# IBM/VillanDiffusion

Measured on AMD Instinct MI355X. Metric: train imgs/sec + 1000-step DDPM sample imgs/sec, CIFAR10 bs128, higher is better.
Workload: dtype bf16x3/f32

## Files before the change

### villandiffusion_amd/csrc/vd_gemm.hip

```cpp
#include "vd_common.h"
#include <string.h>
#include <stdlib.h>

bool vd_conv3_k32p_eligible(const vd_gemm_desc& d);
int vd_launch_conv3_k32p(const vd_gemm_desc& d, int mode, hipStream_t st);
int vd_launch_wgrad_ps_group(const void* jobs, int n, int W, int up, int blocks, hipStream_t st, bool one);
bool vd_conv3_sm_eligible(const vd_gemm_desc& d);
int vd_launch_conv3_sm(const vd_gemm_desc& d, hipStream_t st);
bool vd_gemm1x1_k32p_pick(const vd_gemm_desc& d);
int vd_launch_gemm1x1_k32p(const vd_gemm_desc& d, hipStream_t st);

namespace {

constexpr int NT = 256;
constexpr int BK = 32;
constexpr int KG = BK / 4;

struct Pix {
    int b, oy, ox, p;
    bool valid;
};

__device__ __forceinline__ void kdecomp9(int k, int& c, int& r, int& s) {
    c = k / 9;
// ... 881 lines not shown
                    float v = acc[m][j];
#pragma unroll
                    for (int k = 0; k < NW - 1; ++k) v += red[k][m][j][lane];
                    v *= d.alpha;
                    if (d.bias) v += d.bias[m];
                    o[j] = v;
                }
                *reinterpret_cast<f32x4*>(d.D + (int64_t)b * d.d_bstride + (int64_t)m * d.ldd + y * W + 4 * x4) = o;
            }
        }
    }
}

static bool fewout_eligible(const vd_gemm_desc& d) {
    return d.W % 4 == 0 && d.C >= 16 && (d.b_bstride & 3) == 0 && (d.d_bstride & 3) == 0 && (d.ldd & 3) == 0 &&
           ((((uintptr_t)d.B) | ((uintptr_t)d.D)) & 15) == 0 && (int64_t)d.H * d.W == d.NP;
}

static bool smallm_eligible(const vd_gemm_desc& d) {
    if (d.b_mode == VD_B_CONV3_T) {
        if (d.a_mode != VD_A_ROW || d.M > 4 || d.tile != 0 || d.debug != 0 || d.act || d.bias || d.pool2 || d.b_presplit) return false;
        if (d.rowadd || d.residual || d.d_trans || d.accumulate || d.bias_on_n || d.nb2 > 1 || d.a_bstride != 0 || d.gn_ss) return false;
        return d.OH == d.H && d.OW == d.W && d.lda == d.K && d.K == d.C * 9 && fewout_eligible(d);
    }
    if (d.b_mode != VD_B_CONV3 || d.a_mode != VD_A_ROW || d.M > 4 || d.tile != 0 || d.debug != 0 || d.act) return false;
    if (d.rowadd || d.residual || d.d_trans || d.accumulate || d.bias_on_n || d.nb2 > 1 || d.a_bstride != 0 || d.gn_ss) return false;
    if (d.OH != d.H || d.OW != d.W) return false;
    if (d.W % 32 == 0) return d.H % 8 == 0;
    return d.W == 16 && d.H % 16 == 0;
}

static int launch_smallm(const vd_gemm_desc& d, hipStream_t st) {
    const int nb = d.N / d.NP;
    if (d.b_mode == VD_B_CONV3_T) {
        const int64_t quads = (int64_t)nb * d.H * (d.W / 4);
        hipLaunchKernelGGL((conv3_fewout_kernel<4, 8, true>), dim3((unsigned)((quads + 63) / 64)), dim3(512), 0, st, d, quads);
        return 0;
    }
    if (fewout_eligible(d)) {
        const int64_t quads = (int64_t)nb * d.H * (d.W / 4);
        hipLaunchKernelGGL((conv3_fewout_kernel<4, 8>), dim3((unsigned)((quads + 63) / 64)), dim3(512), 0, st, d, quads);
        return 0;
    }
    if (d.W % 32 == 0) {
        dim3 grid((unsigned)(nb * (d.H / 8) * (d.W / 32)));
        hipLaunchKernelGGL((conv3_smallm_kernel<32, 4>), grid, dim3(256), 0, st, d);
    } else {
        dim3 grid((unsigned)(nb * (d.H / 16)));
        hipLaunchKernelGGL((conv3_smallm_kernel<16, 4>), grid, dim3(256), 0, st, d);
    }
    return 0;
}

template <int AMODE>
__global__ __launch_bounds__(NT, 3) void gemm_plain_kernel(const vd_gemm_desc d) {
    constexpr int WM = 2, WN = 2, BM = 128, BN = 128;
    constexpr int LD_ = 128 + 4;
    constexpr int LDA_ = (AMODE == VD_A_ROW) ? 129 : 132;
    constexpr int F4 = BM * BK / 4 / NT;
    __shared__ __attribute__((aligned(16))) float As[BK * LDA_];
    __shared__ __attribute__((aligned(16))) float Bs[BK * LD_];

    const int tid = threadIdx.x, lane = tid & 63, wave = tid >> 6, h = lane >> 5;
    const int tiles_m = (d.M + BM - 1) / BM;
    int bid = blockIdx.x;
    {
        const int nwg = gridDim.x;
        if ((nwg & 7) == 0) bid = (bid & 7) * (nwg >> 3) + (bid >> 3);
    }
    const int tm = bid % tiles_m, tn = bid / tiles_m;
    const int m0 = tm * BM, n0 = tn * BN;
    const int b = n0 / d.NP, p0 = n0 - b * d.NP;
    const float* __restrict__ Ap = d.A + batch_off(d, b, d.a_bstride, d.a_b2stride);
    const float* __restrict__ Bp = d.B + batch_off(d, b, d.b_bstride, d.b_b2stride) + p0;

    f32x4 ra[F4], rb[F4];
    auto load_stage = [&](int k0) {
#pragma unroll
        for (int i = 0; i < F4; ++i) {
            const int idx = tid + i * NT;
            if (AMODE == VD_A_ROW) {
                const int m = idx >> 3, q = idx & 7;
                ra[i] = *reinterpret_cast<const f32x4*>(Ap + (int64_t)min(m0 + m, d.M - 1) * d.lda + k0 + 4 * q);
            } else {
                const int k = idx >> 5, q = idx & 31;
                ra[i] = *reinterpret_cast<const f32x4*>(Ap + (int64_t)(k0 + k) * d.lda + min(m0 + 4 * q, d.M - 4));
            }
            const int k = idx >> 5, q = idx & 31;
            rb[i] = *reinterpret_cast<const f32x4*>(Bp + (int64_t)(k0 + k) * d.ldb + 4 * q);
        }
    };
    auto store_stage = [&]() {
#pragma unroll
        for (int i = 0; i < F4; ++i) {
            const int idx = tid + i * NT;
            if (AMODE == VD_A_ROW) {
                const int m = idx >> 3, q = idx & 7;
                const bool ok = m0 + m < d.M;
#pragma unroll
                for (int j = 0; j < 4; ++j) As[(4 * q + j) * LDA_ + m] = ok ? ra[i][j] : 0.f;
            } else {
                const int k = idx >> 5, q = idx & 31;
                const bool ok = m0 + 4 * q < d.M;
                *reinterpret_cast<f32x4*>(&As[k * LDA_ + 4 * q]) = ok ? ra[i] : f32x4{0.f, 0.f, 0.f, 0.f};
            }
            const int k = idx >> 5, q = idx & 31;
// ... 768 lines not shown
    if (row >= B * M) return;
    const int b = row / M, m = row - b * M;
    const float* __restrict__ x = X + (int64_t)b * x_bs + (int64_t)m * P;
    const int lane = threadIdx.x & 63;
    float s = 0.f;
    if ((P & 3) == 0 && ((((uintptr_t)x) & 15) == 0)) {
        const f32x4* x4 = reinterpret_cast<const f32x4*>(x);
        const int Q = P >> 2;
        int i = lane;
        for (; i + 192 < Q; i += 256) {
            const f32x4 v0 = x4[i], v1 = x4[i + 64], v2 = x4[i + 128], v3 = x4[i + 192];
            s += (v0[0] + v0[1]) + (v0[2] + v0[3]);
            s += (v1[0] + v1[1]) + (v1[2] + v1[3]);
            s += (v2[0] + v2[1]) + (v2[2] + v2[3]);
            s += (v3[0] + v3[1]) + (v3[2] + v3[3]);
        }
        for (; i < Q; i += 64) {
            f32x4 v = x4[i];
            s += (v[0] + v[1]) + (v[2] + v[3]);
        }
    } else {
        for (int i = lane; i < P; i += 64) s += x[i];
    }
    s = wave_sum(s);
    if (lane == 0) ws[(int64_t)b * ws_ld + m] = s;
}

__global__ __launch_bounds__(256) void colsum_kernel(const float* __restrict__ ws, float* __restrict__ out, int B, int C,
                                                     int64_t ld, int accumulate) {
    __shared__ float part[4][64];
    const int lane = threadIdx.x & 63, w = threadIdx.x >> 6;
    const int c = blockIdx.x * 64 + lane;
    float s = 0.f;
    if (c < C) {
        int b = w;
        for (; b + 28 < B; b += 32) {
            float t[8];
#pragma unroll
            for (int u = 0; u < 8; ++u) t[u] = ws[(int64_t)(b + 4 * u) * ld + c];
#pragma unroll
            for (int u = 0; u < 8; ++u) s += t[u];
        }
        for (; b < B; b += 4) s += ws[(int64_t)b * ld + c];
    }
    part[w][lane] = s;
    __syncthreads();
    if (w == 0 && c < C) {
        const float t = (part[0][lane] + part[1][lane]) + (part[2][lane] + part[3][lane]);
        out[c] = accumulate ? (out[c] + t) : t;
    }
}

template <bool BIG_IS_X>
__global__ __launch_bounds__(256) void wgrad_small_kernel(const vd_wgrad_desc d) {
    constexpr int MAXS = 4, PWM = 34;
    __shared__ float S[MAXS * PWM * PWM];
    const int CB = BIG_IS_X ? d.C : d.M, CS = BIG_IS_X ? d.M : d.C;
    const int H = d.OH, W = d.OW, HW = H * W;
    constexpr int PW = PWM, PHW = PWM * PWM;
    const int cb_blocks = (CB + 31) / 32, tiles_x = (W + 31) / 32, tiles = tiles_x * ((H + 31) / 32);
    int rest = blockIdx.x;
    const int cb0 = (rest % cb_blocks) * 32;
    rest /= cb_blocks;
    const int tile = rest % tiles, b = rest / tiles;
    const int y0 = (tile / tiles_x) * 32, x0 = (tile - (tile / tiles_x) * tiles_x) * 32;
    const int TH = min(32, H - y0), TW = min(32, W - x0);
    const float* __restrict__ big = (BIG_IS_X ? d.X + (int64_t)b * d.x_bstride : d.dY + (int64_t)b * d.dy_bstride);
    const float* __restrict__ sml = (BIG_IS_X ? d.dY + (int64_t)b * d.dy_bstride : d.X + (int64_t)b * d.x_bstride);
    for (int i = threadIdx.x; i < CS * PHW; i += 256) {
        const int cs = i / PHW, rem = i - cs * PHW;
        const int yy = y0 + rem / PW - 1, xx = x0 + rem - (rem / PW) * PW - 1;
        const bool ok = (unsigned)yy < (unsigned)H && (unsigned)xx < (unsigned)W;
        S[i] = ok ? sml[(int64_t)cs * HW + yy * W + xx] : 0.f;
    }
    __syncthreads();
    const int x = threadIdx.x & 31, slot = threadIdx.x >> 5;
    const int Ncols = d.C * 9;
    float* __restrict__ part = d.ws + ((int64_t)b * tiles + tile) * d.M * Ncols;
    float acc[4][MAXS][9];
#pragma unroll
    for (int k = 0; k < 4; ++k)
#pragma unroll
        for (int cs = 0; cs < MAXS; ++cs)
#pragma unroll
            for (int t = 0; t < 9; ++t) acc[k][cs][t] = 0.f;
    if (x < TW) {
        const float* __restrict__ src[4];
        bool live[4];
#pragma unroll
        for (int k = 0; k < 4; ++k) {
            const int cb = cb0 + slot + 8 * k;
            live[k] = cb < CB;
            src[k] = big + (int64_t)(live[k] ? cb : 0) * HW + (int64_t)y0 * W + x0 + x;
        }
        for (int y = 0; y < TH; ++y) {
            float v[4];
#pragma unroll
            for (int k = 0; k < 4; ++k) v[k] = src[k][y * W];
#pragma unroll
            for (int k = 0; k < 4; ++k) v[k] = live[k] ? v[k] : 0.f;
#pragma unroll
            for (int cs = 0; cs < MAXS; ++cs) {
                if (cs < CS) {
                    const float* __restrict__ sp = S + cs * PHW + (y + 1) * PW + (x + 1);
#pragma unroll
                    for (int t = 0; t < 9; ++t) {
                        const int r = t / 3, sx = t - 3 * r;
                        const int dy = BIG_IS_X ? 1 - r : r - 1, dx = BIG_IS_X ? 1 - sx : sx - 1;
                        const float sv = sp[dy * PW + dx];
#pragma unroll
                        for (int k = 0; k < 4; ++k) acc[k][cs][t] = fmaf(v[k], sv, acc[k][cs][t]);
                    }
                }
            }
        }
    }
#pragma unroll
    for (int k = 0; k < 4; ++k) {
        const int cb = cb0 + slot + 8 * k;
        if (cb >= CB) continue;
#pragma unroll
        for (int cs = 0; cs < MAXS; ++cs) {
            if (cs < CS) {
#pragma unroll
                for (int t = 0; t < 9; ++t) {
                    float v = acc[k][cs][t];
#pragma unroll
                    for (int off = 16; off > 0; off >>= 1) v += __shfl_xor(v, off, 32);
                    if (x == 0) {
                        const int m = BIG_IS_X ? cs : cb, c = BIG_IS_X ? cb : cs;
                        part[(int64_t)m * Ncols + c * 9 + t] = v;
                    }
                }
            }
        }
    }
}

static bool wgrad_small_eligible(const vd_wgrad_desc& d) {
    if (d.T != 9 || d.mode != VD_B_CONV3 || d.tile != 0 || d.math != 0) return false;
    if (d.H != d.OH || d.W != d.OW || d.OH * d.OW != d.NP) return false;
    const bool small_m = d.M <= 4 && d.C >= 32, small_c = d.C <= 4 && d.M >= 32;
    return (small_m || small_c) && d.nb >= 1;
}
static int wgrad_small_parts(const vd_wgrad_desc& d) { return d.nb * vd_cdiv(d.OW, 32) * vd_cdiv(d.OH, 32); }

__global__ __launch_bounds__(256) void colsum_seg_kernel(const int64_t* __restrict__ table, int B) {
    __shared__ float part[4][64];
    const int64_t* __restrict__ t = table + 4 * (int64_t)blockIdx.x;
    const float* __restrict__ ws = reinterpret_cast<const float*>(t[0]);
    float* __restrict__ out = reinterpret_cast<float*>(t[1]);
    const int C = (int)t[2];
    const int64_t ld = t[3];
    const int lane = threadIdx.x & 63, w = threadIdx.x >> 6;
    const int c = lane;
    float s = 0.f;
    if (c < C) {
        int b = w;
        for (; b + 28 < B; b += 32) {
            float v[8];
#pragma unroll
            for (int u = 0; u < 8; ++u) v[u] = ws[(int64_t)(b + 4 * u) * ld + c];
#pragma unroll
            for (int u = 0; u < 8; ++u) s += v[u];
        }
        for (; b < B; b += 4) s += ws[(int64_t)b * ld + c];
    }
    part[w][lane] = s;
    __syncthreads();
    if (w == 0 && c < C) out[c] += (part[0][lane] + part[1][lane]) + (part[2][lane] + part[3][lane]);
}

template <int WM, int WN>
int launch_gemm_t(const vd_gemm_desc& d, hipStream_t st) {
    constexpr int BM = 64 * WM, BN = 64 * WN;
    const int grid = vd_cdiv(d.M, BM) * vd_cdiv(d.N, BN);
#define VD_GEMM_CASE(AM, BMD)                                                                   \
    if (d.a_mode == AM && d.b_mode == BMD) {                                                    \
        hipLaunchKernelGGL((gemm_kernel<WM, WN, AM, BMD>), dim3(grid), dim3(NT), 0, st, d);     \
        return 0;                                                                               \
    }
    VD_GEMM_CASE(VD_A_ROW, VD_B_PLAIN)
    VD_GEMM_CASE(VD_A_ROW, VD_B_KCONTIG)
    VD_GEMM_CASE(VD_A_ROW, VD_B_CONV3)
    VD_GEMM_CASE(VD_A_ROW, VD_B_CONV3_T)
    VD_GEMM_CASE(VD_A_ROW, VD_B_CONV3_S2)
    VD_GEMM_CASE(VD_A_ROW, VD_B_CONV3_UP)
    VD_GEMM_CASE(VD_A_ROW, VD_B_CONV3_DIL)
    VD_GEMM_CASE(VD_A_ROW, VD_B_CONVG)
    VD_GEMM_CASE(VD_A_COL, VD_B_PLAIN)
    VD_GEMM_CASE(VD_A_COL, VD_B_KCONTIG)
// ... 35 lines not shown
    unsigned long long* p = (unsigned long long*)buf;
    return (int)hipMemcpyToSymbol(HIP_SYMBOL(g_wg_stamps), &p, sizeof(p));
}
#endif

extern "C" int64_t vd_gemm_ws_floats(const vd_gemm_desc* desc) {
    if (desc && desc->a_packed) {
        const int tile = vd_gemm_tile(desc);
        int splits = 1, per;
        if (tile == 9) gemm_bx3_plan(*desc, splits, per);
        else if (tile == 8 || tile == 16) bx3_plan(*desc, splits, per);
        return splits > 1 ? (int64_t)splits * desc->M * desc->N : 0;
    }
    if (!desc || !patch_eligible(*desc)) return 0;
    int splits, ks_per;
    patch_plan(*desc, splits, ks_per);
    return splits > 1 ? (int64_t)splits * desc->M * desc->N : 0;
}

extern "C" int vd_gemm_tile(const vd_gemm_desc* desc) {
    if (!desc) return 0;
    const vd_gemm_desc& d = *desc;
    if (d.a_packed && d.math == 2) {
        if (bx3_eligible(d) && !bx3_big_split(d) && k32p_pick(d)) return 18;
        if (gemm_bx3_eligible(d) && vd_gemm1x1_k32p_pick(d)) return 19;
        return -1;
    }
    if (d.a_packed && d.math == 3) {
        if (bx3_eligible(d)) {
            if (vd_conv3_sm_eligible(d)) return 20;
            if (!bx3_big_split(d) && k32p_pick(d)) return 18;
            return -1;
        }
        if (gemm_bx3_eligible(d) && vd_gemm1x1_k32p_pick(d)) return 19;
        return -1;
    }
    if (d.a_packed) {
        if (bx3_eligible(d)) {
            if (vd_conv3_sm_eligible(d)) return 20;
            if (bx3_big_split(d)) return 16;
            if (k32p_pick(d)) return 18;
            int splits, c_per;
            bx3_plan(d, splits, c_per);
            const int big = d.b_mode == VD_B_CONV3_S2 ? 0 : bx3_big_tile(d, splits);
            return big == 2 ? 15 : (big == 1 ? 12 : 8);
        }
        if (!gemm_bx3_eligible(d)) return -1;
        if (vd_gemm1x1_k32p_pick(d)) return 19;
        if (gemm_bx3_big_tile(d)) return 13;
        return vd_cdiv(d.M, 128) * (d.N / 128) >= 1024 ? 11 : 9;
    }
    if (d.math == 1) return gemm_bx3_act_eligible(d) ? 10 : -1;
    if (smallm_eligible(d)) return 7;
    if (patch_eligible(d)) {
        int splits, ks_per;
        patch_plan(d, splits, ks_per);
        return (splits == 1 && patch_wide(d)) ? 6 : 4;
    }
    if (plain_eligible(d)) return 5;
    int max_bn = 128;
    if (d.a_bstride != 0 && d.NP % 128 != 0) max_bn = 64;
    int tile = d.tile ? d.tile : pick_tile(d.M, d.N, max_bn);
    if (max_bn < 128 && tile != 3) tile = 3;
    return tile;
}

extern "C" int vd_gemm(const vd_gemm_desc* desc, void* stream) {
    VD_REQUIRE(desc != nullptr, "vd_gemm: null desc");
    vd_gemm_desc d = *desc;
    VD_REQUIRE(d.A && d.B && d.D, "vd_gemm: null operand");
    VD_REQUIRE(d.math != 3 || d.a_packed, "vd_gemm: math = 3 (one bf16 product per term) reads the hi plane of a_packed; a_packed is NULL");
#ifndef VD_ABLATION
    VD_REQUIRE(d.debug == 0, "vd_gemm: desc.debug = %d -- timing-only ablation bits exist in `make ABLATION=1` builds only", d.debug);
#endif
    VD_REQUIRE(d.M > 0 && d.N > 0 && d.K > 0 && d.NP > 0 && d.N % d.NP == 0, "vd_gemm: bad dims M=%d N=%d K=%d NP=%d", d.M,
               d.N, d.K, d.NP);
    if (d.b_mode >= VD_B_CONV3) {
        VD_REQUIRE(d.C > 0 && d.H > 0 && d.W > 0 && d.OH * d.OW == d.NP, "vd_gemm: bad conv dims");
        if (d.b_mode == VD_B_CONVG)
            VD_REQUIRE(d.kh > 0 && d.kw > 0 && d.K == d.C * d.kh * d.kw && d.conv_stride >= 1 && d.conv_stride <= 4 && d.pad_h >= 0 && d.pad_w >= 0 &&
                           d.OH == (d.H + 2 * d.pad_h - d.kh) / d.conv_stride + 1 && d.OW == (d.W + 2 * d.pad_w - d.kw) / d.conv_stride + 1 &&
                           !d.a_packed && d.math == 0 && d.a_mode == VD_A_ROW,
                       "vd_gemm: VD_B_CONVG needs kh, kw > 0, K = C*kh*kw, conv_stride 1 .. 4, OH / OW = (H + 2 pad - k) / stride + 1, row-major exact-f32 A");
        else
            VD_REQUIRE(d.K == d.C * 9, "vd_gemm: conv K must be C*9");
    }
    VD_REQUIRE(d.act == 0 || (d.act == 1 && !d.a_packed && d.math == 0), "vd_gemm: act = 1 (ReLU) is honoured by the exact-f32 kernels only");
    if (d.a_bstride != 0) VD_REQUIRE(d.NP % 64 == 0, "vd_gemm: per-batch A needs NP %% 64 == 0 (NP=%d)", d.NP);
    VD_REQUIRE(!(d.d_trans && (d.residual || d.rowadd)), "vd_gemm: d_trans excludes residual/rowadd");
    if (d.nb2 > 1)
        VD_REQUIRE(!d.residual && !d.rowadd && !d.d_trans && d.b_mode <= VD_B_KCONTIG && (d.N / d.NP) % d.nb2 == 0,
                   "vd_gemm: two-level batch (nb2=%d) needs plain operands, no residual/rowadd, nb %% nb2 == 0", d.nb2);
    const int tile = vd_gemm_tile(&d);
    VD_REQUIRE(tile != -1, "vd_gemm: a_packed (split-precision bf16) needs a 3x3 convolution with 8x8 / 16x16 / 32x32 outputs, "
                           "C %% 16 == 0, M >= 64, or a VD_B_PLAIN product with shared A, NP %% 128 == 0, K %% 16 == 0, M >= 64; "
                           "a_packed_mpad = M rounded up to 128; math = 1 needs per-batch A, PLAIN / KCONTIG B, NP %% 128 == 0, K %% 16 == 0, K >= 32, M >= 64; "
                           "math = 2 / 3 need the persistent 16x16x32 kernels (vd_gemm_tile 18 / 19; math = 3 also 20)");
    VD_REQUIRE(d.b_presplit == 0 || (d.b_presplit == 1 && tile == 18),
               "vd_gemm: a pre-split B operand (b_presplit = %d) is read by the persistent 16x16x32 convolution only (vd_gemm_tile() == 18; this problem: %d)",
               d.b_presplit, tile);
    VD_REQUIRE(!d.gn_ss || tile == 4 || tile == 6 || tile == 8 || tile == 12 || tile == 15 || tile == 18,
               "vd_gemm: gn_ss (GroupNorm folded into the loader) needs the patch-staged 3x3 kernel (OW 16/32, C %% 8 == 0, M >= 64)");
    VD_REQUIRE(!d.pool2 || tile == 8 || tile == 12 || tile == 18, "vd_gemm: pool2 needs the split-precision 3x3 kernel (VD_B_CONV3_T with a_packed)");
    VD_REQUIRE(!d.act_out || (tile == 18 && d.gn_ss), "vd_gemm: act_out is written by the persistent 16x16x32 3x3 convolution with gn_ss only (vd_gemm_tile() == 18)");
    VD_REQUIRE(!d.gn_part || (tile == 18 && !d.pool2),
               "vd_gemm: gn_part is written by the persistent 16x16x32 split-precision 3x3 kernel only (vd_gemm_tile() == 18)");
    hipStream_t st = (hipStream_t)stream;
    int rc;
    switch (tile) {
        case 1: rc = launch_gemm_t<2, 2>(d, st); break;
        case 2: rc = launch_gemm_t<1, 2>(d, st); break;
        case 3: rc = launch_gemm_t<1, 1>(d, st); break;
        case 4:
        case 6: rc = launch_patch(d, st); break;
        case 7: rc = launch_smallm(d, st); break;
        case 8: case 12: case 15: case 16: case 18: rc = launch_bx3(d, tile, st); break;
        case 19: rc = vd_launch_gemm1x1_k32p(d, st) == 0 ? 0 : VD_EINVAL; break;
        case 20: rc = vd_launch_conv3_sm(d, st) == 0 ? 0 : VD_EINVAL; break;
        case 10: launch_gemm_bx3_act(d, st); rc = 0; break;
        case 13:
            hipLaunchKernelGGL(gemm_bx3_kernel<512>, dim3(vd_cdiv(d.M, 128) * (d.N / 256)), dim3(512), 0, st, d, 1 << 30);
            rc = 0;
            break;
        case 9: {
            int splits, st_per;
            gemm_bx3_plan(d, splits, st_per);
            VD_REQUIRE(splits == 1 || d.ws, "vd_gemm: split-K 1x1 launch needs the workspace (vd_gemm_ws_floats)");
            hipLaunchKernelGGL(gemm_bx3_kernel<256>, dim3(vd_cdiv(d.M, 128) * (d.N / 128), splits), dim3(NT), 0, st, d, st_per);
            if (splits > 1) launch_splitk_epilogue(d, splits, st);
            rc = 0;
            break;
        }
        case 11:
            hipLaunchKernelGGL(gemm_bx3_persist_kernel, dim3(512), dim3(NT), 0, st, d, vd_cdiv(d.M, 128) * (d.N / 128));
            rc = 0;
            break;
        case 5: {
            const int grid = vd_cdiv(d.M, 128) * (d.N / 128);
            if (d.a_mode == VD_A_ROW)
                hipLaunchKernelGGL((gemm_plain_kernel<VD_A_ROW>), dim3(grid), dim3(NT), 0, st, d);
            else
                hipLaunchKernelGGL((gemm_plain_kernel<VD_A_COL>), dim3(grid), dim3(NT), 0, st, d);
            rc = 0;
            break;
        }
        default: vd_set_error("vd_gemm: bad tile %d", tile); return VD_EINVAL;
    }
    if (rc) return rc;
    VD_LAUNCH_CHECK("vd_gemm");
    return 0;
}

extern "C" int64_t vd_conv3_packed_bytes(int M, int C, int taps) {
    if (M <= 0 || C <= 0 || C % XC != 0 || (taps != 9 && taps != 1)) return 0;
    return (int64_t)((M + 127) / 128 * 128) * C * taps * 4;
}

extern "C" int vd_conv3_pack_weights(const float* W, void* packed, int M, int C, int taps, int64_t row_stride, int64_t chan_stride,
                                     void* stream) {
    VD_REQUIRE(W && packed && M > 0 && C > 0 && C % XC == 0 && (taps == 9 || taps == 1),
               "vd_conv3_pack_weights: bad arguments (M=%d C=%d taps=%d; C %% 16 == 0, taps 9 or 1)", M, C, taps);
    VD_REQUIRE((((uintptr_t)packed) & 15) == 0, "vd_conv3_pack_weights: packed must be 16-byte aligned");
    const int Mpad = (M + 127) / 128 * 128;
    const int total = (C / XC) * 2 * Mpad;
    hipLaunchKernelGGL(conv3_pack_kernel, dim3(vd_cdiv(total, 256)), dim3(256), 0, (hipStream_t)stream, W,
                       reinterpret_cast<u32x4*>(packed), M, C, Mpad, row_stride, chan_stride, taps);
    VD_LAUNCH_CHECK("vd_conv3_pack_weights");
    return 0;
// ... 86 lines not shown
    } while (0)
                if (d.mode == VD_B_CONV3_S2) {
                    if (d.OW >= 64) hipLaunchKernelGGL((wgrad_bx3_kernel<32, 4, true>), grid, dim3(NT), 0, st, d, kk_per);
                    else if (d.OW == 32) hipLaunchKernelGGL((wgrad_bx3_kernel<32, 4>), grid, dim3(NT), 0, st, d, kk_per);
                    else if (d.OW == 16) hipLaunchKernelGGL((wgrad_bx3_kernel<16, 4>), grid, dim3(NT), 0, st, d, kk_per);
                    else hipLaunchKernelGGL((wgrad_bx3_kernel<8, 4>), grid, dim3(NT), 0, st, d, kk_per);
                } else if (d.OW >= 64 && up) hipLaunchKernelGGL((wgrad_bx3_kernel<32, 2, true>), grid, dim3(NT), 0, st, d, kk_per);
                else if (d.OW >= 64) hipLaunchKernelGGL((wgrad_bx3_kernel<32, 0, true>), grid, dim3(NT), 0, st, d, kk_per);
                else if (d.OW == 4) hipLaunchKernelGGL((wgrad_bx3_kernel<4, 0>), grid, dim3(NT), 0, st, d, kk_per);
                else if (d.OW == 32) VD_WK32(32);
                else if (d.OW == 16) VD_WK32(16);
                else VD_WK32(8);
#undef VD_WK32
            } else if (wgrad_patch_kind(d) == 3) {
                const int ohs = ilog2_exact(d.OH);
                const bool up = d.mode == VD_B_CONV3_UP;
                if (d.OW == 32) {
                    if (up) hipLaunchKernelGGL((wgrad_patch_gen_kernel<2, 2, 64>), grid, dim3(NT), 0, st, d, kk_per, ohs, 0);
                    else hipLaunchKernelGGL((wgrad_patch_gen_kernel<2, 0, 64>), grid, dim3(NT), 0, st, d, kk_per, ohs, 0);
                } else {
                    if (up) hipLaunchKernelGGL((wgrad_patch_gen_kernel<4, 2, 64>), grid, dim3(NT), 0, st, d, kk_per, ohs, 0);
                    else hipLaunchKernelGGL((wgrad_patch_gen_kernel<4, 0, 64>), grid, dim3(NT), 0, st, d, kk_per, ohs, 0);
                }
            } else if (wgrad_patch_kind(d) == 2) {
                const int ohs = ilog2_exact(d.OH), sgs = d.OW >= 32 ? ilog2_exact(d.OW / 32) : 0;
                const bool up = d.mode == VD_B_CONV3_UP;
#define VD_WPG(R_)                                                                                               \
    do {                                                                                                         \
        if (up)                                                                                                  \
            hipLaunchKernelGGL((wgrad_patch_gen_kernel<R_, 2, 32>), grid, dim3(NT), 0, st, d, kk_per, ohs, sgs);     \
        else                                                                                                     \
            hipLaunchKernelGGL((wgrad_patch_gen_kernel<R_, 0, 32>), grid, dim3(NT), 0, st, d, kk_per, ohs, sgs);     \
    } while (0)
                if (d.OW == 4)
                    VD_WPG(8);
                else if (d.OW == 8)
                    VD_WPG(4);
                else
                    VD_WPG(1);
#undef VD_WPG
            } else if (d.OW == 32 && d.mode == VD_B_CONV3)
                hipLaunchKernelGGL((wgrad_patch_kernel<32, 0>), grid, dim3(NT), 0, st, d, kk_per);
            else if (d.OW == 32)
                hipLaunchKernelGGL((wgrad_patch_kernel<32, 2>), grid, dim3(NT), 0, st, d, kk_per);
            else if (d.mode == VD_B_CONV3)
                hipLaunchKernelGGL((wgrad_patch_kernel<16, 0>), grid, dim3(NT), 0, st, d, kk_per);
            else
                hipLaunchKernelGGL((wgrad_patch_kernel<16, 2>), grid, dim3(NT), 0, st, d, kk_per);
            break;
        }
        case 6: {
            const int parts = wgrad_small_parts(d);
            const dim3 grid(parts * vd_cdiv(d.M <= 4 ? d.C : d.M, 32));
            if (d.M <= 4) hipLaunchKernelGGL((wgrad_small_kernel<true>), grid, dim3(256), 0, st, d);
            else hipLaunchKernelGGL((wgrad_small_kernel<false>), grid, dim3(256), 0, st, d);
            VD_LAUNCH_CHECK("vd_conv_wgrad/direct");
            hipLaunchKernelGGL(colsum_kernel, dim3(vd_cdiv(d.M * Ncols, 64)), dim3(256), 0, st, d.ws, d.dW, parts, d.M * Ncols,
                               (int64_t)d.M * Ncols, d.accumulate);
            VD_LAUNCH_CHECK("vd_conv_wgrad/direct-reduce");
            return 0;
        }
        case 5:
            hipLaunchKernelGGL(wgrad1x1_bx3_kernel, dim3(vd_cdiv(d.M, 128) * vd_cdiv(d.C, 128), splits), dim3(NT), 0, st, d, kk_per);
            rc = 0;
            break;
        case 1: rc = launch_wgrad_t<2, 2>(d, splits, kk_per, st); break;
        case 2: rc = launch_wgrad_t<1, 2>(d, splits, kk_per, st); break;
        case 3: rc = launch_wgrad_t<1, 1>(d, splits, kk_per, st); break;
        default: vd_set_error("vd_conv_wgrad: bad tile %d", tile); return VD_EINVAL;
    }
    if (rc) return rc;
    VD_LAUNCH_CHECK("vd_conv_wgrad");
    if (splits > 1 && tile == 4) {
        const int64_t n = (int64_t)d.M * Ncols;
        const int grid = (int)((n + 255) / 256 < 4096 ? (n + 255) / 256 : 4096);
        hipLaunchKernelGGL(slab_reduce_perm_kernel, dim3(grid), dim3(256), 0, st, d.ws, d.dW, d.M, d.C, splits, d.accumulate);
        VD_LAUNCH_CHECK("vd_conv_wgrad/reduce");
    } else if (splits > 1) {
        const int64_t n = (int64_t)d.M * Ncols;
        if ((n & 3) == 0 && ((((uintptr_t)d.dW) & 15) == 0) && ((((uintptr_t)d.ws) & 15) == 0)) {
            const int grid = (int)((n / 4 + 255) / 256 < 2048 ? (n / 4 + 255) / 256 : 2048);
            hipLaunchKernelGGL(slab_reduce_kernel, dim3(grid), dim3(256), 0, st, d.ws, d.dW, n / 4, splits, d.accumulate);
        } else {
            const int grid = (int)((n + 255) / 256 < 2048 ? (n + 255) / 256 : 2048);
            hipLaunchKernelGGL(slab_reduce_scalar_kernel, dim3(grid), dim3(256), 0, st, d.ws, d.dW, n, splits, d.accumulate);
        }
        VD_LAUNCH_CHECK("vd_conv_wgrad/reduce");
    }
    return 0;
}

constexpr int VD_WG_ONE = 10000;
static int wgrad_group_class(const vd_wgrad_desc& d) {
    if (d.math == 3) {
        vd_wgrad_desc d1 = d;
        d1.math = 1;
        const int c = wgrad_group_class(d1);
        const int v = c ? vd_conv_wgrad_group_variant(c) : 0;
        return (v == 3000 || v == 32 || v == 256) ? VD_WG_ONE + c : 0;
    }
    if (d.math != 1 || d.splits != 0 || d.tile != 0) return 0;
    if (d.presplit != 0) {
        const bool up = d.mode == VD_B_CONV3_UP;
        if (d.presplit != 3 || d.T != 9 || (d.mode != VD_B_CONV3 && !up) || (d.OW != 8 && d.OW != 16 && d.OW != 32) || d.OH != d.OW ||
            d.H * (up ? 2 : 1) != d.OH || d.W * (up ? 2 : 1) != d.OW ||
            (d.M & 7) || (d.C & 7) || d.M < 64 || d.C < 64 || (d.dy_bstride & 3) || (d.x_bstride & 3) || ((((uintptr_t)d.dY) | ((uintptr_t)d.X)) & 15) ||
            (int64_t)d.M * d.NP * 4 >= (1ll << 32) || (int64_t)d.C * d.NP * 4 >= (1ll << 32))
            return 0;
// ... 236 lines not shown
```

### villandiffusion_amd/flops.py

```python
from __future__ import annotations

from typing import Dict


def unet_forward_flops(net, breakdown: bool = False):
    S = net.sample_size
    f: Dict[str, float] = {"conv3x3": 0.0, "upsample_conv": 0.0, "downsample_conv": 0.0, "conv1x1_shortcut": 0.0, "attn_proj": 0.0,
                           "attn_core": 0.0, "linear": 0.0, "conv_in_out": 0.0}

    def res(r, hw):
        f["conv3x3"] += 2.0 * 9 * (r.cin * r.cout + r.cout * r.cout) * hw
        if r.has_sc:
            f["conv1x1_shortcut"] += 2.0 * r.cin * r.cout * hw
        f["linear"] += 2.0 * net.temb_dim * r.cout

    def attn(a, hw):
        f["attn_proj"] += 2.0 * (3 * a.ch * a.ch + a.ch * a.ch) * hw
        f["attn_core"] += 2.0 * 2 * hw * hw * a.ch

    f["linear"] += 2.0 * (net.time_dim0 * net.temb_dim + net.temb_dim * net.temb_dim)
    f["conv_in_out"] += 2.0 * 9 * net.in_channels * net._conv_in.cout * S * S
    s = S
    for blk in net.down:
        for j, r in enumerate(blk["res"]):
            res(r, s * s)
            if blk["attn"]:
                attn(blk["attn"][j], s * s)
        if blk["ds"] is not None:
            s //= 2
            f["downsample_conv"] += 2.0 * 9 * blk["ds"].cin * blk["ds"].cout * s * s
    for r in net.mid_res:
        res(r, s * s)
    attn(net.mid_attn, s * s)
    for blk in net.up:
        for j, r in enumerate(blk["res"]):
            res(r, s * s)
            if blk["attn"]:
                attn(blk["attn"][j], s * s)
        if blk["us"] is not None:
            s *= 2
            f["upsample_conv"] += 2.0 * 9 * blk["us"].cin * blk["us"].cout * s * s
    f["conv_in_out"] += 2.0 * 9 * net._conv_out.cin * net.out_channels * S * S
    total = sum(f.values())
    return (total, f) if breakdown else total


SPLIT_PRECISION_FAMILIES = ("bx3", "attn_core", "attn_flash", "k32", "wgrad9", "wgrad1x1_wide", "wgrad_ps", "presplit", "conv3_sm")
EXACT_F32_FAMILIES = ("gemm_kernel<", "gemm_plain_kernel", "conv3_patch_kernel", "wgrad_patch_kernel", "wgrad_patch_gen_kernel", "wgrad_kernel<",
                      "wgrad_small_kernel", "conv3_fewout_kernel", "conv3_smallm_kernel", "attn_small")


def is_split_precision(kernel_name: str) -> bool:
    if any(f in kernel_name for f in SPLIT_PRECISION_FAMILIES):
        return True
    if any(f in kernel_name for f in EXACT_F32_FAMILIES):
        return False
    raise KeyError(f"matrix kernel {kernel_name!r} is in neither SPLIT_PRECISION_FAMILIES nor EXACT_F32_FAMILIES (villandiffusion_amd/flops.py)")
```

### villandiffusion_amd/ops.py

```python
from __future__ import annotations

import ctypes as C
import math
import os
from typing import Optional, Sequence

import torch

from . import lib as L
from .lib import (A_COL, A_ROW, B_CONV3, B_CONV3_DIL, B_CONVG, B_CONV3_S2, B_CONV3_T, B_CONV3_UP, B_KCONTIG, B_PLAIN,
                  GemmDesc, WgradDesc)


def _lib():
    L.require_device()
    return L.load()


_PROF = None

_B_NAMES = {0: "PLAIN", 1: "KCONTIG", 2: "CONV3", 3: "CONV3_T", 4: "CONV3_S2", 5: "CONV3_UP", 6: "CONV3_DIL", 7: "CONVG"}
_TILE_NAMES = {1: "128x128", 2: "64x128", 3: "64x64", 4: "patch128x128"}


# ... 229 lines not shown
    if a_packed16 is not None and (gn_part is None or alt_math == 3):
        d.a_packed, d.math = a_packed16.data_ptr(), alt_math
        if lib.vd_gemm_tile(C.byref(d)) not in ((18, 19) if alt_math == 2 else (18, 19, 20)):
            d.a_packed, d.math = a_packed.data_ptr(), math_mode
    LAST_GEMM_MATH = d.math
    LAST_GEMM_TILE = lib.vd_gemm_tile(C.byref(d))
    GN_PART_WRITTEN = gn_part is not None and not pool2 and LAST_GEMM_TILE == 18
    if GN_PART_WRITTEN:
        assert gn_part.is_contiguous() and gn_part.numel() >= (N // 256) * M * 2
        d.gn_part = gn_part.data_ptr()
    if _PROF is None:
        L.check(lib.vd_gemm(C.byref(d), _s()), "vd_gemm")
        return D
    e0, e1 = torch.cuda.Event(enable_timing=True), torch.cuda.Event(enable_timing=True)
    e0.record()
    L.check(lib.vd_gemm(C.byref(d), _s()), "vd_gemm")
    e1.record()
    flops = 2.0 * M * N * K * (0.25 if b_mode == B_CONV3_DIL else 1.0)
    if conv is not None:
        nb_ = N // d.NP
        b_elems = nb_ * d.C * d.H * d.W
        a_elems = M * K
    else:
        b_elems = K * N
        a_elems = M * K * (N // d.NP if a_bstride else 1)
    d_elems = M * N // (4 if pool2 else 1)
    nbytes = 4.0 * (b_elems + d_elems * (2 if residual is not None else 1) + a_elems)
    tl = LAST_GEMM_TILE
    if tl == 10:
        name = f"gemm_bx3_act_kernel<{int(a_mode == A_ROW)}, {int(b_mode == B_KCONTIG)}>"
    elif tl == 19:
        big = d.math != 2 and M % 256 == 0 and N % 128 == 0
        name = ("gemm1x1_k32p_kernel<true, 128>" if d.math == 2 else
                f"gemm1x1_k32p_kernel<false, {256 if big else 128}{', true' if d.math == 3 else ''}>")
    elif tl in (9, 11, 13):
        name = "gemm_bx3_persist_kernel" if tl == 11 else f"gemm_bx3_kernel<{512 if tl == 13 else 256}>"
    elif tl == 18:
        md = (3 if gn_ss is not None else 0) if b_mode == B_CONV3 else (1 if b_mode == B_CONV3_T else 2)
        name = (f"conv3_k32p_kernel<{16 if d.OW == 16 else 32}, {md}, true, true, {'true' if d.math == 2 else 'false'}, {'true' if d.b_presplit else 'false'}"
                + (", true>" if d.math == 3 else ">")
                + (f"@{d.OW}" if d.OW > 32 else ""))
    elif tl == 20:
        imgs = 2 if d.OW == 8 else 4
        name = f"conv3_sm_kernel<{d.OW}, {1 if b_mode == B_CONV3_T else 0}, {imgs}, 1{', true' if d.math == 3 else ''}>"
    elif tl in (8, 12, 15, 16):
        md = (3 if gn_ss is not None else 0) if b_mode == B_CONV3 else (1 if b_mode == B_CONV3_T else (4 if b_mode == B_CONV3_S2 else 2))
        name = f"conv3_bx3_kernel<{d.OW if d.OW <= 64 else 128}, {md}, {4 if tl == 15 else 2}, {256 if tl == 8 else 512}, 2>"
    elif tl in (4, 6):
        tw = d.OW if d.OW <= 64 else 128
        md = (3 if gn_ss is not None else 0) if b_mode == B_CONV3 else (1 if b_mode == B_CONV3_T else (4 if b_mode == B_CONV3_S2 else 2))
        name = f"conv3_patch_kernel<{tw}, {md}, {4 if tl == 6 else 2}>"
    elif tl == 5:
        name = f"gemm_plain_kernel<{a_mode}>"
    elif tl == 7:
        few = d.W % 4 == 0 and d.C >= 16 and d.b_bstride % 4 == 0 and d.d_bstride % 4 == 0 and d.ldd % 4 == 0
        name = (f"conv3_fewout_kernel<4, 8, {'true' if b_mode == B_CONV3_T else 'false'}>" if few or b_mode == B_CONV3_T
                else f"conv3_smallm_kernel<{32 if d.W % 32 == 0 else 16}, 4>")
    else:
        name = f"gemm_kernel<{_TILE_NAMES[tl]},{'ROW' if a_mode == A_ROW else 'COL'},{_B_NAMES[b_mode]}>"
    _PROF.append({"name": name, "flops": flops, "bytes": nbytes, "e0": e0, "e1": e1, "kind": "mfma", "shape": (M, K, d.NP, N // d.NP, d.OH, d.OW)})
    return D


_CONV_OUT = {B_CONV3: lambda h, w: (h, w), B_CONV3_T: lambda h, w: (h, w), B_CONV3_S2: lambda h, w: (h // 2, w // 2),
             B_CONV3_UP: lambda h, w: (2 * h, 2 * w), B_CONV3_DIL: lambda h, w: (2 * h, 2 * w)}


def conv3_pack_weights(w2d, M, Cc, transposed=False, out=None, taps=9):
    lib = _lib()
    nbytes = lib.vd_conv3_packed_bytes(M, Cc, taps)
    assert nbytes > 0, (M, Cc, taps)
    if out is None:
        out = torch.empty(nbytes // 4, device=w2d.device, dtype=torch.int32)
    assert out.numel() * out.element_size() >= nbytes and w2d.is_contiguous()
    rs, cs = (taps, M * taps) if transposed else (Cc * taps, taps)
    L.check(lib.vd_conv3_pack_weights(_p(w2d), _p(out), M, Cc, taps, rs, cs, _s()), "vd_conv3_pack_weights")
    return out


def conv3_pack_weights_f16(w2d, M, Cc, transposed=False, taps=9):
    nbytes = _lib().vd_conv3_packed_bytes(M, Cc, taps) // 2
    assert nbytes > 0 and w2d.is_contiguous(), (M, Cc, taps)
    out = torch.empty(nbytes // 4, device=w2d.device, dtype=torch.int32)
    rs, cs = (taps, M * taps) if transposed else (Cc * taps, taps)
    mpad = (M + 127) // 128 * 128
    tab = torch.tensor([[w2d.data_ptr(), out.data_ptr(), M, Cc, rs, cs, 0, taps]], dtype=torch.int64).to(w2d.device)
    conv3_pack_weights_f16_multi(tab, 1, (mpad * (Cc // 16) * 2 + 255) // 256)
    torch.cuda.current_stream(w2d.device).synchronize()
    return out


def conv3_pack_weights_f16_multi(table, n_jobs, total_blocks):
    assert table.dtype == torch.int64 and table.is_contiguous() and table.numel() >= 8 * n_jobs
    L.check(_lib().vd_conv3_pack_weights_f16_multi(_p(table), n_jobs, total_blocks, _s()), "vd_conv3_pack_weights_f16_multi")


def conv3_pack_weights_multi(table, n_jobs, total_blocks):
    assert table.dtype == torch.int64 and table.is_contiguous() and table.numel() >= 8 * n_jobs
    L.check(_lib().vd_conv3_pack_weights_multi(_p(table), n_jobs, total_blocks, _s()), "vd_conv3_pack_weights_multi")


WEIGHTS_EPOCH = 0


def bx3_eligible(M, Cc, OH, OW, mode) -> bool:
    if mode == B_CONV3_S2:
# ... 242 lines not shown
        ws_ptr = ws.data_ptr()
        table = upload_table(torch.frombuffer(bytearray(host), dtype=torch.uint8), device,
                             after=lambda t: L.check(lib.vd_conv_wgrad_group_rebase(t.data_ptr(), n, ws_ptr, _s()), "vd_conv_wgrad_group_rebase"))
        if len(_WG_CACHE) > 256:
            _WG_CACHE.clear()
        ent = _WG_CACHE[key] = {"table": table, "cls": cls, "blocks": blocks.value, "rblocks": rblocks.value, "ws_ptr": ws.data_ptr(),
                                "ws_floats": int(wsf.value)}
    if _CAPTURE_TABLES is not None:
        _CAPTURE_TABLES.append(ent["table"])
    flops = sum(2.0 * d.M * d.C * d.T * d.nb * d.NP for d in descs)
    nbytes = sum(4.0 * (d.nb * d.M * d.NP + d.nb * d.C * d.H * d.W + d.M * d.C * d.T) for d in descs)
    var = lib.vd_conv_wgrad_group_variant(ent["cls"])
    if ent["cls"] > WGRAD_ONE:
        bc = ent["cls"] - WGRAD_ONE
        if bc >= 3000:
            name = f"wgrad_ps_group_kernel<{(bc - 3000) // 4}, {(bc - 3000) & 2}, true>(+group_reduce)"
        elif bc == 1000:
            name = "wgrad1x1_wide_group_kernel<true>(+group_reduce)"
        else:
            name = f"wgrad_k32_group_kernel<{bc // 4}, {bc & 2}, true>(+group_reduce)"
    elif ent["cls"] >= 3000:
        name = f"wgrad_ps_group_kernel<{(ent['cls'] - 3000) // 4}, {(ent['cls'] - 3000) & 2}>(+group_reduce)"
    elif ent["cls"] > 2000:
        name = "wgrad_bx3_group_kernel<32, 4, true>(+group_reduce)" if ent["cls"] == 2033 else f"wgrad_bx3_group_kernel<{ent['cls'] - 2000}, 4, false>(+group_reduce)"
    elif ent["cls"] == 1000:
        name = "wgrad1x1_wide_group_kernel(+group_reduce)"
    elif var == 32:
        name = f"wgrad_k32_group_kernel<{ent['cls'] // 4}, {ent['cls'] & 2}>(+group_reduce)"
    else:
        name = f"wgrad_bx3_group_kernel<{ent['cls'] // 4}, {ent['cls'] & 2}, {'true' if ent['cls'] & 1 else 'false'}>(+group_reduce)"
    _timed(name, flops, "mfma", lambda: L.check(
        lib.vd_conv_wgrad_group_launch(ent["table"].data_ptr(), n, ent["cls"], ent["blocks"], ent["rblocks"], _s()), "vd_conv_wgrad_group_launch"),
        nbytes=nbytes)


def conv_wgrad(dy, x, dw2d, mode, ws: Optional[torch.Tensor], accumulate=False, splits=0, tile=0, pad=0, math_mode=0):
    d = wgrad_desc(dy, x, dw2d, mode, ws, accumulate, splits, tile, pad, math_mode)
    Bn, M, OH, OW = dy.shape
    Cc, T = x.shape[1], d.T
    lib = _lib()
    need = lib.vd_conv_wgrad_ws_floats(C.byref(d))
    if need > 0:
        assert ws is not None and ws.numel() >= need, f"wgrad workspace too small: need {need}"
    if _PROF is None:
        L.check(lib.vd_conv_wgrad(C.byref(d), _s()), "vd_conv_wgrad")
        return dw2d
    e0, e1 = torch.cuda.Event(enable_timing=True), torch.cuda.Event(enable_timing=True)
    e0.record()
    L.check(lib.vd_conv_wgrad(C.byref(d), _s()), "vd_conv_wgrad")
    e1.record()
    tl, sp = C.c_int32(0), C.c_int32(0)
    lib.vd_conv_wgrad_plan(C.byref(d), C.byref(tl), C.byref(sp))
    if tl.value == 6:
        name = f"wgrad_small_kernel<{'true' if M <= 4 else 'false'}>(+colsum)"
    elif tl.value == 5:
        name = "wgrad1x1_bx3_kernel(+slab_reduce)"
    elif tl.value == 4 and math_mode == 1:
        name = f"wgrad_bx3_kernel<{min(OW, 32)}, {0 if mode == B_CONV3 else 2}{', wide' if OW > 32 else ''}>(+slab_reduce)"
    elif tl.value == 4:
        name = f"wgrad_patch_kernel<{OW}, {0 if mode == B_CONV3 else 2}>(+slab_reduce)"
    else:
        name = f"wgrad_kernel<{_TILE_NAMES[tl.value]},{_B_NAMES[mode]}>(+slab_reduce)"
    _PROF.append({"name": name, "flops": 2.0 * M * Cc * T * Bn * OH * OW, "bytes": 4.0 * (dy.numel() + x.numel() + M * Cc * T),
                  "e0": e0, "e1": e1, "kind": "mfma"})
    return dw2d


def _wgrad_s2_split(OW) -> bool:
    sel = os.environ.get("VILLAN_WGRAD_S2", "all")
    return sel == "all" or (sel != "none" and OW >= 32)


def wgrad_bx3_eligible(M, Cc, OH, OW, mode) -> bool:
    if mode == B_PLAIN:
        return (OH * OW) % 8 == 0 and M >= 64 and Cc >= 64
    if (mode == B_CONV3 and OW == 4 and OH == 4) or (mode in (B_CONV3, B_CONV3_UP) and OW >= 64 and OW % 32 == 0):
        return M >= 64 and Cc >= 64
    if mode == B_CONV3_S2:
        return OH == OW and (OW in (8, 16, 32) or (OW >= 64 and OW % 32 == 0)) and M >= 64 and Cc >= 64 and _wgrad_s2_split(OW)
    return mode in (B_CONV3, B_CONV3_UP) and OH == OW and OW in (8, 16, 32) and M >= 64 and Cc >= 64


def wgrad_ws_floats(M, Cc, T, nb, NP, OH=None, OW=None, mode=None, math_mode=0) -> int:
    d = WgradDesc()
    if OH is None:
        OH = OW = int(round(math.sqrt(NP)))
    d.M, d.C, d.T, d.nb, d.NP, d.OH, d.OW = M, Cc, T, nb, NP, OH, OW
    d.mode = (B_PLAIN if T == 1 else B_CONV3) if mode is None else mode
    d.math = math_mode
    scale = {B_CONV3_UP: (1, 2), B_CONV3_S2: (2, 1)}.get(d.mode, (1, 1))
    d.H, d.W = OH * scale[0] // scale[1], OW * scale[0] // scale[1]
    return int(L.load().vd_conv_wgrad_ws_floats(C.byref(d)))


def weight_transpose(w2d, wt, M, Cc, T):
    L.check(_lib().vd_weight_transpose(_p(w2d), _p(wt), M, Cc, T, _s()), "vd_weight_transpose")
    return wt


def sumpool2x2(dU, dX, accumulate=False):
    Bn, Cc, H, W, xbs = _img(dX)
    ubs = _img(dU)[4]
    assert dU.shape == (Bn, Cc, 2 * H, 2 * W)
    L.check(_lib().vd_sumpool2x2(_p(dU), _p(dX), Bn, Cc, H, W, ubs, xbs, int(accumulate), _s()), "vd_sumpool2x2")
    return dX


# ... 371 lines not shown
```

Measured before the change: 7600.

## Add direct few-input-channel conv3 kernel and vectorized small wgrad kernel

```diff
diff --git a/villandiffusion_amd/csrc/vd_gemm.hip b/villandiffusion_amd/csrc/vd_gemm.hip
--- a/villandiffusion_amd/csrc/vd_gemm.hip
+++ b/villandiffusion_amd/csrc/vd_gemm.hip
@@ -957,6 +957,113 @@
     return 0;
 }
 
+template <int CC, bool FLIP>
+__global__ __launch_bounds__(256) void conv3_fewin_kernel(const vd_gemm_desc d, int64_t quads, int mper) {
+    constexpr int K = CC * 9;
+    const int lane = threadIdx.x & 63, wave = __builtin_amdgcn_readfirstlane(threadIdx.x >> 6);
+    const int W = d.W, H = d.H, W4 = W >> 2, HWs = H * W;
+    const int64_t gq = ((int64_t)blockIdx.x * 4 + wave) * 64 + lane;
+    const bool live = gq < quads;
+    const int64_t g = live ? gq : 0;
+    const int x4 = (int)(g % W4);
+    const int64_t rest = g / W4;
+    const int y = (int)(rest % H), b = (int)(rest / H);
+    const float* __restrict__ xb = d.B + (int64_t)b * d.b_bstride + y * W + 4 * x4;
+    const bool rowok[3] = {y > 0, true, y < H - 1};
+    const bool lf = x4 > 0, rt = x4 < W4 - 1;
+    const bool xch = W4 <= 16 && (64 % W4) == 0;
+    float e[CC][3][6];
+#pragma unroll
+    for (int c = 0; c < CC; ++c)
+#pragma unroll
+        for (int r = 0; r < 3; ++r) {
+            const float* __restrict__ q = xb + (int64_t)c * HWs + (rowok[r] ? (r - 1) * W : 0);
+            const f32x4 v = *reinterpret_cast<const f32x4*>(q);
+            const float l = xch ? __shfl_up(v[3], 1) : q[lf ? -1 : 0], rr = xch ? __shfl_down(v[0], 1) : q[rt ? 4 : 3];
+            e[c][r][0] = (rowok[r] && lf) ? l : 0.f;
+            e[c][r][5] = (rowok[r] && rt) ? rr : 0.f;
+#pragma unroll
+            for (int j = 0; j < 4; ++j) e[c][r][1 + j] = rowok[r] ? v[j] : 0.f;
+        }
+    const int m_begin = blockIdx.y * mper, m_end = min(d.M, m_begin + mper);
+    float* __restrict__ out = d.D + (int64_t)b * d.d_bstride + y * W + 4 * x4;
+    auto ldw = [&](int m, float (&dst)[K]) {
+        const float* __restrict__ wm = d.A + (int64_t)m * d.lda;
+#pragma unroll
+        for (int k = 0; k < K; ++k) dst[k] = wm[k];
+    };
+    auto channel = [&](int m, const float (&wc)[K], float bc) {
+        float acc[4] = {0.f, 0.f, 0.f, 0.f};
+#pragma unroll
+        for (int kb = 0; kb < (K + 7) / 8; ++kb)
+#pragma unroll
+            for (int t = 0; t < 4; ++t)
+#pragma unroll
+                for (int hh = 0; hh < 2; ++hh) {
+                    const int k = 8 * kb + 4 * hh + t;
+                    if (k < K) {
+                        const int c = k / 9, r = (k - 9 * c) / 3, s = k - 9 * c - 3 * r;
+#pragma unroll
+                        for (int j = 0; j < 4; ++j) acc[j] = fmaf(wc[k], e[c][FLIP ? 2 - r : r][(FLIP ? 2 - s : s) + j], acc[j]);
+                    }
+                }
+        f32x4 o;
+#pragma unroll
+        for (int j = 0; j < 4; ++j) o[j] = __fmul_rn(d.alpha, acc[j]);
+        if (d.bias) {
+#pragma unroll
+            for (int j = 0; j < 4; ++j) o[j] = __fadd_rn(o[j], bc);
+        }
+        if (live) *reinterpret_cast<f32x4*>(out + (int64_t)m * d.ldd) = o;
+    };
+    const int m_last = m_end - 1;
+    float wa[K], wb[K], ba = 0.f, bb = 0.f;
+    ldw(m_begin, wa);
+    if (d.bias) ba = d.bias[m_begin];
+    for (int m = m_begin; m < m_end; m += 2) {
+        ldw(min(m + 1, m_last), wb);
+        if (d.bias) bb = d.bias[min(m + 1, m_last)];
+        channel(m, wa, ba);
+        ldw(min(m + 2, m_last), wa);
+        if (d.bias) ba = d.bias[min(m + 2, m_last)];
+        if (m + 1 < m_end) channel(m + 1, wb, bb);
+    }
+}
+
+static bool fewin_eligible(const vd_gemm_desc& d) {
+    if (d.b_mode != VD_B_CONV3 && d.b_mode != VD_B_CONV3_T) return false;
+    if (d.a_mode != VD_A_ROW || d.C < 1 || d.C > 4 || d.M < 32 || d.tile != 0 || d.debug != 0 || d.act || d.pool2 || d.b_presplit) return false;
+    if (d.a_packed || d.math != 0 || d.rowadd || d.residual || d.d_trans || d.accumulate || d.bias_on_n || d.nb2 > 1 || d.a_bstride != 0 || d.gn_ss) return false;
+    if (d.OH != d.H || d.OW != d.W || d.K != d.C * 9 || d.lda < d.K || (int64_t)d.H * d.W != d.NP) return false;
+    return d.W % 4 == 0 && (d.b_bstride & 3) == 0 && (d.d_bstride & 3) == 0 && (d.ldd & 3) == 0 && ((((uintptr_t)d.B) | ((uintptr_t)d.D)) & 15) == 0;
+}
+
+static int launch_fewin(const vd_gemm_desc& d, hipStream_t st) {
+    const int nb = d.N / d.NP;
+    const int64_t quads = (int64_t)nb * d.H * (d.W / 4);
+    const int64_t wgs = (quads + 255) / 256;
+    int slices = (int)((8192 + 4 * wgs - 1) / (4 * wgs));
+    if (slices > vd_cdiv(d.M, 8)) slices = vd_cdiv(d.M, 8);
+    const int mper = vd_cdiv(d.M, slices);
+    slices = vd_cdiv(d.M, mper);
+    const dim3 grid((unsigned)wgs, (unsigned)slices);
+    const bool flip = d.b_mode == VD_B_CONV3_T;
+#define VD_FEWIN(CC_)                                                                                         \
+    case CC_:                                                                                                 \
+        if (flip) hipLaunchKernelGGL((conv3_fewin_kernel<CC_, true>), grid, dim3(256), 0, st, d, quads, mper); \
+        else hipLaunchKernelGGL((conv3_fewin_kernel<CC_, false>), grid, dim3(256), 0, st, d, quads, mper);     \
+        break;
+    switch (d.C) {
+        VD_FEWIN(1)
+        VD_FEWIN(2)
+        VD_FEWIN(3)
+        VD_FEWIN(4)
+        default: return VD_EINVAL;
+    }
+#undef VD_FEWIN
+    return 0;
+}
+
 template <int AMODE>
 __global__ __launch_bounds__(NT, 3) void gemm_plain_kernel(const vd_gemm_desc d) {
     constexpr int WM = 2, WN = 2, BM = 128, BN = 128;
@@ -1831,7 +1938,7 @@
 }
 
 template <bool BIG_IS_X>
-__global__ __launch_bounds__(256) void wgrad_small_kernel(const vd_wgrad_desc d) {
+__global__ __launch_bounds__(256) void wgrad_small_scalar_kernel(const vd_wgrad_desc d) {
     constexpr int MAXS = 4, PWM = 34;
     __shared__ float S[MAXS * PWM * PWM];
     const int CB = BIG_IS_X ? d.C : d.M, CS = BIG_IS_X ? d.M : d.C;
@@ -1916,6 +2023,136 @@
     }
 }
 
+template <int CTRL, int ROW_MASK>
+__device__ __forceinline__ float dpp_add(float v) {
+    return v + __builtin_bit_cast(float, __builtin_amdgcn_update_dpp(0, __builtin_bit_cast(int, v), CTRL, ROW_MASK, 0xF, false));
+}
+__device__ __forceinline__ float half_wave_sum_hi(float v) {
+    v = dpp_add<0xB1, 0xF>(v);
+    v = dpp_add<0x4E, 0xF>(v);
+    v = dpp_add<0x141, 0xF>(v);
+    v = dpp_add<0x140, 0xF>(v);
+    return dpp_add<0x142, 0xA>(v);
+}
+
+template <bool BIG_IS_X>
+__global__ __launch_bounds__(256, 2) void wgrad_small_kernel(const vd_wgrad_desc d) {
+    constexpr int MAXS = 4, PH = 34, PW = 36, PHW = PH * PW, IT = 8, DEPTH = 3;
+    __shared__ __attribute__((aligned(16))) float S[MAXS * PHW];
+    const int CB = BIG_IS_X ? d.C : d.M, CS = BIG_IS_X ? d.M : d.C;
+    const int H = d.OH, W = d.OW, HW = H * W;
+    const int cb_blocks = (CB + 31) / 32, tiles_x = (W + 31) / 32, tiles = tiles_x * ((H + 31) / 32);
+    int rest = blockIdx.x;
+    const int cb0 = (rest % cb_blocks) * 32;
+    rest /= cb_blocks;
+    const int tile = rest % tiles, b = rest / tiles;
+    const int y0 = (tile / tiles_x) * 32, x0 = (tile - (tile / tiles_x) * tiles_x) * 32;
+    const int TH = min(32, H - y0), TW = min(32, W - x0);
+    const float* __restrict__ big = (BIG_IS_X ? d.X + (int64_t)b * d.x_bstride : d.dY + (int64_t)b * d.dy_bstride);
+    const float* __restrict__ sml = (BIG_IS_X ? d.dY + (int64_t)b * d.dy_bstride : d.X + (int64_t)b * d.x_bstride);
+    const int l32 = threadIdx.x & 31, slot = threadIdx.x >> 5;
+    const int x4 = l32 & 7, yq = l32 >> 3;
+    const bool colok = 4 * x4 < TW;
+    const float* __restrict__ src[4];
+    bool live[4];
+#pragma unroll
+    for (int k = 0; k < 4; ++k) {
+        const int cb = cb0 + slot + 8 * k;
+        live[k] = cb < CB && colok;
+        src[k] = big + (int64_t)(cb < CB ? cb : 0) * HW + (int64_t)y0 * W + x0 + (colok ? 4 * x4 : 0);
+    }
+    f32x4 buf[DEPTH][4];
+    auto load = [&](int it, f32x4 (&dst)[4]) {
+        const int y = yq + 4 * it;
+        const int off = y < TH ? y * W : 0;
+#pragma unroll
+        for (int k = 0; k < 4; ++k) dst[k] = *reinterpret_cast<const f32x4*>(src[k] + off);
+    };
+#pragma unroll
+    for (int it = 0; it < DEPTH - 1; ++it) load(it, buf[it]);
+    for (int i = threadIdx.x; i < CS * PHW; i += 256) {
+        const int cs = i / PHW, rem = i - cs * PHW;
+        const int yy = y0 + rem / PW - 1, xx = x0 + rem - (rem / PW) * PW - 1;
+        const bool ok = (unsigned)yy < (unsigned)H && (unsigned)xx < (unsigned)W;
+        S[i] = ok ? sml[(int64_t)cs * HW + yy * W + xx] : 0.f;
+    }
+    __syncthreads();
+    const int Ncols = d.C * 9;
+    float* __restrict__ part = d.ws + ((int64_t)b * tiles + tile) * d.M * Ncols;
+    float acc[4][MAXS][9];
+#pragma unroll
+    for (int k = 0; k < 4; ++k)
+#pragma unroll
+        for (int cs = 0; cs < MAXS; ++cs)
+#pragma unroll
+            for (int t = 0; t < 9; ++t) acc[k][cs][t] = 0.f;
+#pragma unroll
+    for (int it = 0; it < IT; ++it) {
+        if (it + DEPTH - 1 < IT) load(it + DEPTH - 1, buf[(it + DEPTH - 1) % DEPTH]);
+        const int y = yq + 4 * it;
+        const bool rok = y < TH;
+        f32x4 v[4];
+#pragma unroll
+        for (int k = 0; k < 4; ++k) v[k] = sel4(rok && live[k], buf[it % DEPTH][k]);
+#pragma unroll
+        for (int cs = 0; cs < MAXS; ++cs) {
+            if (cs < CS) {
+                const float* __restrict__ sp = S + cs * PHW + y * PW + 4 * x4;
+                float e[3][6];
+#pragma unroll
+                for (int r = 0; r < 3; ++r) {
+                    const f32x4 a = *reinterpret_cast<const f32x4*>(sp + r * PW);
+                    const float2 c2 = *reinterpret_cast<const float2*>(sp + r * PW + 4);
+                    e[r][0] = a[0], e[r][1] = a[1], e[r][2] = a[2], e[r][3] = a[3], e[r][4] = c2.x, e[r][5] = c2.y;
+                }
+#pragma unroll
+                for (int t = 0; t < 9; ++t) {
+                    const int r = t / 3, sx = t - 3 * r;
+                    const int dy = BIG_IS_X ? 1 - r : r - 1, dx = BIG_IS_X ? 1 - sx : sx - 1;
+#pragma unroll
+                    for (int j = 0; j < 4; ++j) {
+                        const float sv = e[dy + 1][j + dx + 1];
+#pragma unroll
+                        for (int k = 0; k < 4; ++k) acc[k][cs][t] = fmaf(v[k][j], sv, acc[k][cs][t]);
+                    }
+                }
+            }
+        }
+    }
+#pragma unroll
+    for (int cs = 0; cs < MAXS; ++cs) {
+        if (cs < CS) {
+#pragma unroll
+            for (int k = 0; k < 4; ++k)
+#pragma unroll
+                for (int t = 0; t < 9; ++t) acc[k][cs][t] = half_wave_sum_hi(acc[k][cs][t]);
+        }
+    }
+    if (l32 == 16) {
+#pragma unroll
+        for (int k = 0; k < 4; ++k) {
+            const int cb = cb0 + slot + 8 * k;
+            if (cb < CB) {
+#pragma unroll
+                for (int cs = 0; cs < MAXS; ++cs) {
+                    if (cs < CS) {
+                        const int m = BIG_IS_X ? cs : cb, c = BIG_IS_X ? cb : cs;
+#pragma unroll
+                        for (int t = 0; t < 9; ++t) part[(int64_t)m * Ncols + c * 9 + t] = acc[k][cs][t];
+                    }
+                }
+            }
+        }
+    }
+}
+
+static bool wgrad_small_vec(const vd_wgrad_desc& d) {
+    const bool big_is_x = d.M <= 4;
+    const float* big = big_is_x ? d.X : d.dY;
+    const int64_t bs = big_is_x ? d.x_bstride : d.dy_bstride;
+    return d.OW % 4 == 0 && (bs & 3) == 0 && (((uintptr_t)big) & 15) == 0;
+}
+
 static bool wgrad_small_eligible(const vd_wgrad_desc& d) {
     if (d.T != 9 || d.mode != VD_B_CONV3 || d.tile != 0 || d.math != 0) return false;
     if (d.H != d.OH || d.W != d.OW || d.OH * d.OW != d.NP) return false;
@@ -2057,6 +2294,7 @@
     }
     if (d.math == 1) return gemm_bx3_act_eligible(d) ? 10 : -1;
     if (smallm_eligible(d)) return 7;
+    if (fewin_eligible(d)) return 21;
     if (patch_eligible(d)) {
         int splits, ks_per;
         patch_plan(d, splits, ks_per);
@@ -2119,6 +2357,7 @@
         case 4:
         case 6: rc = launch_patch(d, st); break;
         case 7: rc = launch_smallm(d, st); break;
+        case 21: rc = launch_fewin(d, st); break;
         case 8: case 12: case 15: case 16: case 18: rc = launch_bx3(d, tile, st); break;
         case 19: rc = vd_launch_gemm1x1_k32p(d, st) == 0 ? 0 : VD_EINVAL; break;
         case 20: rc = vd_launch_conv3_sm(d, st) == 0 ? 0 : VD_EINVAL; break;
@@ -2311,8 +2550,13 @@
         case 6: {
             const int parts = wgrad_small_parts(d);
             const dim3 grid(parts * vd_cdiv(d.M <= 4 ? d.C : d.M, 32));
-            if (d.M <= 4) hipLaunchKernelGGL((wgrad_small_kernel<true>), grid, dim3(256), 0, st, d);
-            else hipLaunchKernelGGL((wgrad_small_kernel<false>), grid, dim3(256), 0, st, d);
+            if (wgrad_small_vec(d)) {
+                if (d.M <= 4) hipLaunchKernelGGL((wgrad_small_kernel<true>), grid, dim3(256), 0, st, d);
+                else hipLaunchKernelGGL((wgrad_small_kernel<false>), grid, dim3(256), 0, st, d);
+            } else {
+                if (d.M <= 4) hipLaunchKernelGGL((wgrad_small_scalar_kernel<true>), grid, dim3(256), 0, st, d);
+                else hipLaunchKernelGGL((wgrad_small_scalar_kernel<false>), grid, dim3(256), 0, st, d);
+            }
             VD_LAUNCH_CHECK("vd_conv_wgrad/direct");
             hipLaunchKernelGGL(colsum_kernel, dim3(vd_cdiv(d.M * Ncols, 64)), dim3(256), 0, st, d.ws, d.dW, parts, d.M * Ncols,
                                (int64_t)d.M * Ncols, d.accumulate);
diff --git a/villandiffusion_amd/flops.py b/villandiffusion_amd/flops.py
--- a/villandiffusion_amd/flops.py
+++ b/villandiffusion_amd/flops.py
@@ -47,7 +47,7 @@
 
 SPLIT_PRECISION_FAMILIES = ("bx3", "attn_core", "attn_flash", "k32", "wgrad9", "wgrad1x1_wide", "wgrad_ps", "presplit", "conv3_sm")
 EXACT_F32_FAMILIES = ("gemm_kernel<", "gemm_plain_kernel", "conv3_patch_kernel", "wgrad_patch_kernel", "wgrad_patch_gen_kernel", "wgrad_kernel<",
-                      "wgrad_small_kernel", "conv3_fewout_kernel", "conv3_smallm_kernel", "attn_small")
+                      "wgrad_small_kernel", "wgrad_small_scalar_kernel", "conv3_fewout_kernel", "conv3_fewin_kernel", "conv3_smallm_kernel", "attn_small")
 
 
 def is_split_precision(kernel_name: str) -> bool:
diff --git a/villandiffusion_amd/ops.py b/villandiffusion_amd/ops.py
--- a/villandiffusion_amd/ops.py
+++ b/villandiffusion_amd/ops.py
@@ -305,6 +305,8 @@
         name = f"conv3_patch_kernel<{tw}, {md}, {4 if tl == 6 else 2}>"
     elif tl == 5:
         name = f"gemm_plain_kernel<{a_mode}>"
+    elif tl == 21:
+        name = f"conv3_fewin_kernel<{d.C}, {'true' if b_mode == B_CONV3_T else 'false'}>"
     elif tl == 7:
         few = d.W % 4 == 0 and d.C >= 16 and d.b_bstride % 4 == 0 and d.d_bstride % 4 == 0 and d.ldd % 4 == 0
         name = (f"conv3_fewout_kernel<4, 8, {'true' if b_mode == B_CONV3_T else 'false'}>" if few or b_mode == B_CONV3_T
@@ -653,7 +655,9 @@
     tl, sp = C.c_int32(0), C.c_int32(0)
     lib.vd_conv_wgrad_plan(C.byref(d), C.byref(tl), C.byref(sp))
     if tl.value == 6:
-        name = f"wgrad_small_kernel<{'true' if M <= 4 else 'false'}>(+colsum)"
+        big = x if M <= 4 else dy
+        vec = OW % 4 == 0 and big.stride(0) % 4 == 0 and big.data_ptr() % 16 == 0
+        name = f"wgrad_small{'' if vec else '_scalar'}_kernel<{'true' if M <= 4 else 'false'}>(+colsum)"
     elif tl.value == 5:
         name = "wgrad1x1_bx3_kernel(+slab_reduce)"
     elif tl.value == 4 and math_mode == 1:
```

After: 7566. About the same (-0.4%).
